# gnsscusdr/CU-SDR-Collection

Measured on AMD Instinct MI355X. Metric: IF Msamples/s through tracking correlators; x real-time @ 12-ch GPS L1 C/A, higher is better.
Workload: dtype f32 accumulate over int8 I/Q samples; f64/64-bit fixed-point code+carrier phase; 1 GPU; GPS L1 C/A, 12 channels/GPU, 1-ms E/P/L correlators, 60 s of int8 I/Q IF at 18 Msps (2.16 GB in HBM), batched replay of 719976 blocks per step; channels_per_gpu=12, epochs=59998

## Files before the change

cu-sdr-collection_amd/csrc/corr_common.h:

```cpp
#pragma once
#include <type_traits>

#include "gc_internal.h"


namespace gcorr {

constexpr int kWG = 256;
constexpr int kSPL = 8;

enum Mode { I8_IQ = 0, I8_QI, I16_IQ, I16_QI, I8_REAL, I16_REAL };

constexpr int kInlineBlocks = 16;
constexpr int kGuard = 16;

template <int ARMS>
struct ArmPitch {
  static constexpr int v = ARMS == 1 ? 1 : ARMS == 2 ? 2 : 4;
};
inline int gc_arm_pitch(int arms) { return arms <= 1 ? 1 : arms == 2 ? 2 : 4; }

constexpr int kLaneWaves = 16;

constexpr int kLaneReseedSteps = 128;

__host__ __device__ inline unsigned int gc_tie_window_units(double max_ramp, int lane_steps) {
  const int drift = lane_steps <= kLaneReseedSteps ? lane_steps : kLaneReseedSteps + lane_steps / kLaneReseedSteps + 1;
  return 2u + (unsigned int)drift + (unsigned int)(max_ramp * (16.0 * 2.220446049250313e-16 * 4294967296.0));
}

__host__ __device__ inline unsigned int gc_tie_window_units6(double max_ramp, int lane_steps, double m6) {
  const int drift = lane_steps <= kLaneReseedSteps ? lane_steps : kLaneReseedSteps + lane_steps / kLaneReseedSteps + 1;
  return (unsigned int)(m6 * (double)(4 + drift)) + 8u + (unsigned int)(max_ramp * (16.0 * 2.220446049250313e-16 * 4294967296.0));
}

struct TaggedSlot {
  double value;
  unsigned int tag;
  unsigned int zero;
};

struct InlineBlocks {
  gc_block b[kInlineBlocks];
};

struct DevLoopArgs;

struct KArgs {
  const uint8_t* if_base;
  const gc_block* blocks;
  const DevChannel* chans;
  double* out;
  double* partial;
  double fs;
  double inv_fs;
  int64_t nblocks;
  int splits;
  int xcd_swizzle;
  int red_off;
  int bpw;
  int stride;
  TaggedSlot* tagged;
  unsigned int notify_tag;
  int use_inline;
  const struct DevLoopArgs* devloop;
  int wide;
  long long total_wg;
  int share_el;
  int derived;
  int rho_off;
};

struct Fx {
  int k0;
  unsigned long long G;
};

__device__ __forceinline__ unsigned long long frac_to_u64(double g) {
  const double gh = g * 4294967296.0;
  const unsigned int hi = (unsigned int)gh;
  const double gl = (gh - (double)hi) * 4294967296.0;
  const unsigned int lo = (unsigned int)gl;
  return ((unsigned long long)hi << 32) | lo;
}

__device__ __forceinline__ Fx to_fx(double t) {
  const double kf = ceil(t);
  Fx r;
  r.k0 = (int)kf;
  r.G = frac_to_u64(kf - t);
  return r;
}

template <int MODE>
__device__ __forceinline__ void load_chunk(const uint8_t* __restrict__ base, long long q,
                                           float (&a)[kSPL], float (&b)[kSPL]) {
  if constexpr (MODE == I8_IQ || MODE == I8_QI) {
    const uint4 v = *reinterpret_cast<const uint4*>(base + 16 * q);
    const unsigned int w[4] = {v.x, v.y, v.z, v.w};
#pragma unroll
    for (int j = 0; j < kSPL; ++j) {
      const unsigned int word = w[j >> 1];
      const int sh = (j & 1) * 16;
      const float x0 = (float)(int)(signed char)(word >> sh);
      const float x1 = (float)(int)(signed char)(word >> (sh + 8));
      a[j] = (MODE == I8_IQ) ? x0 : x1;
      b[j] = (MODE == I8_IQ) ? x1 : x0;
    }
  } else if constexpr (MODE == I16_IQ || MODE == I16_QI) {
    const uint4 v0 = *reinterpret_cast<const uint4*>(base + 32 * q);
    const uint4 v1 = *reinterpret_cast<const uint4*>(base + 32 * q + 16);
    const unsigned int w[8] = {v0.x, v0.y, v0.z, v0.w, v1.x, v1.y, v1.z, v1.w};
#pragma unroll
    for (int j = 0; j < kSPL; ++j) {
      const float x0 = (float)(int)(short)(w[j] & 0xffffu);
      const float x1 = (float)(int)(short)(w[j] >> 16);
      a[j] = (MODE == I16_IQ) ? x0 : x1;
      b[j] = (MODE == I16_IQ) ? x1 : x0;
    }
  } else if constexpr (MODE == I8_REAL) {
    const uint2 v = *reinterpret_cast<const uint2*>(base + 8 * q);
    const unsigned int w[2] = {v.x, v.y};
#pragma unroll
    for (int j = 0; j < kSPL; ++j) {
      a[j] = (float)(int)(signed char)(w[j >> 2] >> ((j & 3) * 8));
      b[j] = 0.0f;
    }
  } else {
    const uint4 v = *reinterpret_cast<const uint4*>(base + 16 * q);
    const unsigned int w[4] = {v.x, v.y, v.z, v.w};
#pragma unroll
    for (int j = 0; j < kSPL; ++j) {
      a[j] = (float)(int)(short)((w[j >> 1] >> ((j & 1) * 16)) & 0xffffu);
      b[j] = 0.0f;
    }
  }
}

template <int MODE>
struct Fmt {
  static constexpr int bps = (MODE == I8_IQ || MODE == I8_QI || MODE == I16_REAL) ? 2 : (MODE == I8_REAL) ? 1 : 4;
  static constexpr bool swap = (MODE == I8_QI || MODE == I16_QI);
};

template <int MODE, int SPL>
__device__ __forceinline__ void load_words(const uint8_t* __restrict__ base, long long q,
                                           unsigned int (&w)[SPL * Fmt<MODE>::bps / 4]) {
  constexpr int NW = SPL * Fmt<MODE>::bps / 4;
  const uint8_t* p = base + (long long)(SPL * Fmt<MODE>::bps) * q;
  if constexpr (NW == 2) {
    const uint2 v = *reinterpret_cast<const uint2*>(p);
    w[0] = v.x; w[1] = v.y;
  } else {
#pragma unroll
    for (int k = 0; k < NW / 4; ++k) {
      const uint4 v = *reinterpret_cast<const uint4*>(p + 16 * k);
      w[4 * k] = v.x; w[4 * k + 1] = v.y; w[4 * k + 2] = v.z; w[4 * k + 3] = v.w;
    }
  }
}

template <int MODE, int SPL>
__device__ __forceinline__ void mask_words(unsigned int (&w)[SPL * Fmt<MODE>::bps / 4], int i0, int N) {
  constexpr int bits = 8 * Fmt<MODE>::bps;
  constexpr int per_word = 32 / bits;
#pragma unroll
  for (int j = 0; j < SPL; ++j) {
    const bool valid = (unsigned int)(i0 + j) < (unsigned int)N;
    const unsigned int m = (bits == 32) ? 0xffffffffu : (((1u << bits) - 1u) << ((j % per_word) * bits));
    if (!valid) w[j / per_word] &= ~m;
  }
}

#define GC_CVT_SDWA(sel)                                                                                  \
  {                                                                                                       \
    float r;                                                                                              \
    asm("v_cvt_f32_i32_sdwa %0, sext(%1) dst_sel:DWORD dst_unused:UNUSED_PAD src0_sel:" sel : "=v"(r) : "v"(word)); \
    return r;                                                                                             \
  }
template <int B>
__device__ __forceinline__ float cvt_byte(unsigned int word) {
  if constexpr (B == 0) GC_CVT_SDWA("BYTE_0")
  else if constexpr (B == 1) GC_CVT_SDWA("BYTE_1")
  else if constexpr (B == 2) GC_CVT_SDWA("BYTE_2")
  else GC_CVT_SDWA("BYTE_3")
}
template <int H>
__device__ __forceinline__ float cvt_half(unsigned int word) {
  if constexpr (H == 0) GC_CVT_SDWA("WORD_0")
  else GC_CVT_SDWA("WORD_1")
}

template <int MODE, int J, int NW>
__device__ __forceinline__ void sample_ab(const unsigned int (&w)[NW], float& a, float& b) {
  float x0, x1;
  if constexpr (MODE == I8_IQ || MODE == I8_QI) {
    x0 = cvt_byte<(J & 1) * 2>(w[J >> 1]);
    x1 = cvt_byte<(J & 1) * 2 + 1>(w[J >> 1]);
  } else if constexpr (MODE == I16_IQ || MODE == I16_QI) {
    x0 = cvt_half<0>(w[J]);
    x1 = cvt_half<1>(w[J]);
  } else if constexpr (MODE == I8_REAL) {
    x0 = cvt_byte<J & 3>(w[J >> 2]);
    x1 = 0.0f;
  } else {
    x0 = cvt_half<J & 1>(w[J >> 1]);
    x1 = 0.0f;
  }
  a = Fmt<MODE>::swap ? x1 : x0;
  b = Fmt<MODE>::swap ? x0 : x1;
}

template <int J, int SPL, typename F>
__device__ __forceinline__ void static_for(F&& f) {
  if constexpr (J < SPL) {
    f(std::integral_constant<int, J>{});
    static_for<J + 1, SPL>(f);
  }
}

__device__ __forceinline__ float wave_sum_lane63(float v) {
  auto dpp = [](float x, auto ctrl, auto row_mask) {
    return __int_as_float(__builtin_amdgcn_update_dpp(0, __float_as_int(x), decltype(ctrl)::value,
                                                      decltype(row_mask)::value, 0xf, true));
  };
  v += dpp(v, std::integral_constant<int, 0x111>{}, std::integral_constant<int, 0xf>{});
  v += dpp(v, std::integral_constant<int, 0x112>{}, std::integral_constant<int, 0xf>{});
  v += dpp(v, std::integral_constant<int, 0x114>{}, std::integral_constant<int, 0xf>{});
  v += dpp(v, std::integral_constant<int, 0x118>{}, std::integral_constant<int, 0xf>{});
  v += dpp(v, std::integral_constant<int, 0x142>{}, std::integral_constant<int, 0xa>{});
  v += dpp(v, std::integral_constant<int, 0x143>{}, std::integral_constant<int, 0xc>{});
  return v;
}

#ifndef GC_LANE_PN
#define GC_LANE_PN 1
#endif

__device__ __forceinline__ int wave_transpose_slot(int lane) {
  return ((lane >> 2) & 3) | ((lane & 3) << 2) | (lane & 16);
}
namespace wts {
template <int CTRL>
__device__ __forceinline__ float quad(float x) {
  return __int_as_float(__builtin_amdgcn_update_dpp(0, __float_as_int(x), CTRL, 0xf, 0xf, true));
}
__device__ __forceinline__ float pick(float x, float y, unsigned long long mask) {
  float r;
  asm("v_cndmask_b32_e64 %0, %1, %2, %3" : "=v"(r) : "v"(x), "v"(y), "s"(mask));
  return r;
}
template <int S>
__device__ __forceinline__ float row_pair(float x, float y) {
  float r;
  if constexpr (S == 4)
    asm("s_nop 1\n\tv_add_f32_dpp %0, %1, %1 row_shl:4 row_mask:0xf bank_mask:0x5\n\t"
        "v_add_f32_dpp %0, %2, %2 row_shr:4 row_mask:0xf bank_mask:0xa"
        : "=&v"(r) : "v"(x), "v"(y));
  else
    asm("s_nop 1\n\tv_add_f32_dpp %0, %1, %1 row_shl:8 row_mask:0xf bank_mask:0x3\n\t"
        "v_add_f32_dpp %0, %2, %2 row_shr:8 row_mask:0xf bank_mask:0xc"
        : "=&v"(r) : "v"(x), "v"(y));
  return r;
}
}

template <int K>
__device__ __forceinline__ float wave_transpose_sum(const float (&v)[K], int lane) {
  static_assert(K >= 1 && K <= 32, "one value per lane of half a wave at most");
  constexpr int N1 = (K + 1) / 2, N2 = (N1 + 1) / 2, N3 = (N2 + 1) / 2, N4 = (N3 + 1) / 2;
  constexpr unsigned long long kBit0 = 0xaaaaaaaaaaaaaaaaull, kBit1 = 0xccccccccccccccccull, kBit4 = 0xffff0000ffff0000ull;
  float a1[N1], a2[N2], a3[N3], a4[N4];
#pragma unroll
  for (int i = 0; i < N1; ++i) a1[i] = wts::row_pair<4>(v[2 * i], v[2 * i + 1 < K ? 2 * i + 1 : 2 * i]);
#pragma unroll
  for (int i = 0; i < N2; ++i) a2[i] = wts::row_pair<8>(a1[2 * i], a1[2 * i + 1 < N1 ? 2 * i + 1 : 2 * i]);
#pragma unroll
  for (int i = 0; i < N3; ++i) {
    if (2 * i + 1 < N2)
      a3[i] = wts::pick(a2[2 * i], a2[2 * i + 1], kBit0) + wts::quad<0xB1>(wts::pick(a2[2 * i + 1], a2[2 * i], kBit0));
    else
      a3[i] = a2[2 * i] + wts::quad<0xB1>(a2[2 * i]);
  }
#pragma unroll
  for (int i = 0; i < N4; ++i) {
    if (2 * i + 1 < N3)
      a4[i] = wts::pick(a3[2 * i], a3[2 * i + 1], kBit1) + wts::quad<0x4E>(wts::pick(a3[2 * i + 1], a3[2 * i], kBit1));
    else
      a4[i] = a3[2 * i] + wts::quad<0x4E>(a3[2 * i]);
  }
  float r;
  if constexpr (N4 == 2)
    r = wts::pick(a4[0], a4[1], kBit4) + __int_as_float(__builtin_amdgcn_ds_swizzle(__float_as_int(wts::pick(a4[1], a4[0], kBit4)), 0x401F));
  else
    r = a4[0] + __int_as_float(__builtin_amdgcn_ds_swizzle(__float_as_int(a4[0]), 0x401F));
  return r + __int_as_float(__builtin_amdgcn_ds_bpermute((lane ^ 32) << 2, __float_as_int(r)));
}

__device__ __forceinline__ float rl_f(float v, int lane) {
  return __int_as_float(__builtin_amdgcn_readlane(__float_as_int(v), lane));
}
__device__ __forceinline__ unsigned int rl_u(unsigned int v, int lane) {
  return (unsigned int)__builtin_amdgcn_readlane((int)v, lane);
}


constexpr size_t kInlineOffset = (sizeof(KArgs) + 7) / 8 * 8;

__device__ __forceinline__ gc_block load_block(const KArgs& p, long long lb) {
#if defined(__HIP_DEVICE_COMPILE__)
  if (p.use_inline) {
    typedef const __attribute__((address_space(4))) char* cptr4;
    typedef const __attribute__((address_space(4))) unsigned long long* qptr4;
    qptr4 src = (qptr4)((cptr4)__builtin_amdgcn_kernarg_segment_ptr() + kInlineOffset + lb * sizeof(gc_block));
    union {
      gc_block b;
      unsigned long long q[sizeof(gc_block) / 8];
    } u;
#pragma unroll
    for (int i = 0; i < (int)(sizeof(gc_block) / 8); ++i) u.q[i] = src[i];
    return u.b;
  }
#endif
  return p.blocks[lb];
}


}

int gc_launch_devloop_lane(gc_context* ctx, const gcorr::KArgs& a, const LaunchScope& s, unsigned int grid, bool share_el, int waves);
int gc_launch_correlator_lane(gc_context* ctx, const gcorr::KArgs& a, const gcorr::InlineBlocks& ib, const LaunchScope& s, const LaunchPlan& plan);
int gc_launch_correlator_multi(gc_context* ctx, const gcorr::KArgs& a, const LaunchScope& s, const LaunchPlan& plan);
int gc_launch_correlator_cboc(gc_context* ctx, const gcorr::KArgs& a, const LaunchScope& s, const LaunchPlan& plan);
int gc_launch_devloop(gc_context* ctx, const gcorr::KArgs& a, const LaunchScope& s, unsigned int grid, bool spl16, bool share_el);
int gc_launch_correlator_fast(gc_context* ctx, const gcorr::KArgs& a, const gcorr::InlineBlocks& ib, const LaunchScope& s, const LaunchPlan& plan);
```

cu-sdr-collection_amd/csrc/corr_fast.hip:

```cpp
#include <cstdlib>

#include "corr_common.h"
#include "devloop.h"

using namespace gcorr;

namespace {

constexpr float kTieTol = 4e-6f;
constexpr int kFW = 64;
#ifndef GC_SCHED_GROUP
#define GC_SCHED_GROUP 4
#endif
#ifndef GC_FAST_PARENT_SCHEDULE
#define GC_FAST_PARENT_SCHEDULE 0
#endif

template <int OFF_RE, int OFF_IM>
__device__ __forceinline__ void store_prefix(float tr, float ti, unsigned int lds_base) {
  asm volatile("s_mov_b32 m0, %2\n\ts_nop 0\n\tds_write_addtid_b32 %0 offset:%3\n\tds_write_addtid_b32 %1 offset:%4"
               :
               : "v"(tr), "v"(ti), "s"(lds_base), "n"(OFF_RE), "n"(OFF_IM)
               : "memory", "m0");
}

__device__ __forceinline__ double half_sum_f64(double v) {
  auto dpp64 = [](double x, auto ctrl, auto row_mask) {
    const unsigned long long b = (unsigned long long)__double_as_longlong(x);
    const unsigned int lo = (unsigned int)__builtin_amdgcn_update_dpp(0, (int)(unsigned int)b, decltype(ctrl)::value, decltype(row_mask)::value, 0xf, true);
    const unsigned int hi = (unsigned int)__builtin_amdgcn_update_dpp(0, (int)(unsigned int)(b >> 32), decltype(ctrl)::value, decltype(row_mask)::value, 0xf, true);
    return __longlong_as_double((long long)(((unsigned long long)hi << 32) | lo));
  };
  v += dpp64(v, std::integral_constant<int, 0x111>{}, std::integral_constant<int, 0xf>{});
  v += dpp64(v, std::integral_constant<int, 0x112>{}, std::integral_constant<int, 0xf>{});
  v += dpp64(v, std::integral_constant<int, 0x114>{}, std::integral_constant<int, 0xf>{});
  v += dpp64(v, std::integral_constant<int, 0x118>{}, std::integral_constant<int, 0xf>{});
  v += dpp64(v, std::integral_constant<int, 0x142>{}, std::integral_constant<int, 0xa>{});
  return v;
}
__device__ __forceinline__ double rl_f64(double x, int lane) {
  const unsigned long long b = (unsigned long long)__double_as_longlong(x);
  return __longlong_as_double((long long)(((unsigned long long)(unsigned int)__builtin_amdgcn_readlane((int)(b >> 32), lane) << 32) |
                                          (unsigned int)__builtin_amdgcn_readlane((int)(unsigned int)b, lane)));
}

template <int ARMS, int MODE, int SPL, bool CL, bool SHARE_EL, int WIDE, bool DEVLOOP = false>
__global__ __launch_bounds__(WIDE != 0 ? 256 : kFW) void corr_epl_fast_kernel(const KArgs p, const InlineBlocks ) {
  extern __shared__ __attribute__((aligned(16))) unsigned char smem[];
  constexpr int NW = SPL * Fmt<MODE>::bps / 4;
  constexpr bool kReal = (MODE == I8_REAL || MODE == I16_REAL);
  constexpr int kShift = (SPL == 16) ? 4 : 3;

  long long wg = blockIdx.x;
  if (p.xcd_swizzle && !DEVLOOP) {
    const long long per = (long long)gridDim.x >> 3;
    wg = (wg & 7) * per + (wg >> 3);
    if (wg >= p.total_wg) return;
  }
  const int lane = threadIdx.x & 63;
  const int wave = WIDE != 0 ? __builtin_amdgcn_readfirstlane((int)(threadIdx.x >> 6)) : 0;
  const bool wave_items = WIDE != 0 && p.bpw == 1;
  const long long item = wave_items ? wg * 4 + wave : wg;
  const long long wq = (DEVLOOP && p.xcd_swizzle) ? (item & 7) + 8 * ((item >> 3) / p.splits) : item / p.splits;
  const int split = (DEVLOOP && p.xcd_swizzle) ? (int)((item >> 3) % p.splits) : (int)(item - wq * p.splits);
  const long long grp = wq / p.stride;
  const int cslot = (int)(wq - grp * p.stride);

  constexpr bool TABF = (WIDE == 2);
  float2* tab2[ARMS];
  unsigned short* tab16[ARMS];
  float* tabf[ARMS];
  {
    const long long lb0 = min(grp * p.bpw * p.stride + cslot, (long long)p.nblocks - 1);
    const gc_block blk0 = DEVLOOP ? p.devloop->chan[lb0].blk : CL ? load_block(p, lb0) : p.blocks[lb0];
    const DevChannel* __restrict__ chn0 = p.chans + blk0.channel;
#pragma unroll
    for (int a = 0; a < ARMS; ++a) {
      const int aa = (a < chn0->arms) ? a : 0;
      tab2[a] = reinterpret_cast<float2*>(smem + 8 * (size_t)chn0->lds_off[aa]);
      tab16[a] = reinterpret_cast<unsigned short*>(smem + 2 * (size_t)chn0->lds_off[aa]);
      tabf[a] = reinterpret_cast<float*>(smem + 4 * (size_t)chn0->lds_off[aa]);
      if (a < chn0->arms) {
        const int off = blk0.table_offset[a];
        const int n = min(chn0->stage_len[a], chn0->nent[a] - off);
        if constexpr (TABF) {
          const float2* __restrict__ src = chn0->tab2[a] + off;
#pragma unroll 4
          for (int i = threadIdx.x; i < n + 3; i += 256) tabf[a][i] = src[i].x;
          if (threadIdx.x == 0) tabf[a][n + 3] = 0.0f;
        } else if constexpr (WIDE != 0) {
          const unsigned short* __restrict__ src = chn0->tab2b[a] + off;
#pragma unroll 4
          for (int i = threadIdx.x; i < n + 3; i += 256) tab16[a][i] = src[i];
        } else {
          const float2* __restrict__ src = chn0->tab2[a] + off;
#pragma unroll 4
          for (int i = lane; i < n + 3; i += kFW) tab2[a][i] = src[i];
        }
      }
    }
    __syncthreads();
  }
  auto table_entry = [&](int ar, int k) -> float2 {
    if constexpr (TABF) {
      return make_float2(tabf[ar][k + 1], tabf[ar][k + 2]);
    } else if constexpr (WIDE != 0) {
      const unsigned int e = tab16[ar][k + 1];
      float c, dc;
      asm("v_cvt_f32_i32_sdwa %0, sext(%1) dst_sel:DWORD dst_unused:UNUSED_PAD src0_sel:BYTE_0" : "=v"(c) : "v"(e));
      asm("v_cvt_f32_i32_sdwa %0, sext(%1) dst_sel:DWORD dst_unused:UNUSED_PAD src0_sel:BYTE_1" : "=v"(dc) : "v"(e));
      return make_float2(c, dc);
    } else {
      return tab2[ar][k + 1];
    }
  };
  float* pfx = reinterpret_cast<float*>(smem + p.red_off + (DEVLOOP ? 8 * 3 * 64 : 64)) + (WIDE != 0 ? wave * SPL * 2 * kFW : 0);
  unsigned int pfx_m0 = __builtin_amdgcn_readfirstlane((unsigned int)(size_t)pfx);
  if (wave_items && wq >= p.nblocks) return;

  [[maybe_unused]] DevLoopArgs dl_loc;
  if constexpr (DEVLOOP) dl_loc = *p.devloop;
  int nloop = p.bpw;
  gc_block dl_next;
  (void)dl_next;
  DevLoopChan dl_st;
  if constexpr (DEVLOOP) dl_st = p.devloop->chan[min(wq, (long long)p.nblocks - 1)];
  (void)dl_st;
  if constexpr (DEVLOOP) nloop = dl_st.epoch_budget;
  constexpr int kPfWords = SPL * Fmt<MODE>::bps / 4;
  [[maybe_unused]] unsigned int pf_w[kPfWords];
  [[maybe_unused]] long long pf_off = -1;
  constexpr bool kLoadAfterWait = !CL && !DEVLOOP && GC_FAST_PARENT_SCHEDULE == 0;
  for (int bi = (WIDE != 0 && !wave_items) ? wave : 0; bi < nloop; bi += (WIDE != 0 && !wave_items) ? 4 : 1) {
  const long long lb = DEVLOOP ? wq : (grp * p.bpw + bi) * p.stride + cslot;
  if (lb >= p.nblocks) break;
  gc_block blk;
  if constexpr (DEVLOOP) {
    if (dl_loc.host_loop) {
      const DevLoopArgs* dl = &dl_loc;
      const msg_t* dm = (split == 0 ? dl->host_desc : dl->desc_msg) + lb * kDescWords;
      msg_t m = {0u, 0u, 0u, 0u};
      unsigned int spins = 0;
      while (true) {
        if (lane < kDescWords) m = msg_load(dm + lane);
        const bool ok = lane >= kDescWords || m.z == (unsigned int)bi + 1u || m.z == 0xffffffffu;
        if (__all(ok)) break;
        if (++spins > (1u << 22)) break;
        __builtin_amdgcn_s_sleep(2);
      }
      if (spins > (1u << 22)) {
        if (lane == 0) dl->chan[lb].status = 3;
        if (split == 0 && lane < kDescWords) msg_store(dl->desc_msg + lb * kDescWords + lane, msg_t{3u, 0u, (unsigned int)bi + 1u, 0u});
        break;
      }
      if (split == 0 && lane < kDescWords) msg_store(dl->desc_msg + lb * kDescWords + lane, m);
      union {
        gc_block b;
        unsigned long long q[sizeof(gc_block) / 8];
      } u;
#pragma unroll
      for (int i = 0; i < (int)(sizeof(gc_block) / 8); ++i)
        u.q[i] = ((unsigned long long)(unsigned int)__builtin_amdgcn_readlane((int)m.y, i) << 32) | (unsigned int)__builtin_amdgcn_readlane((int)m.x, i);
      if (__builtin_amdgcn_readlane((int)m.x, kDescWords - 1) != 0) break;
      blk = u.b;
    } else if (bi > 0) {
      blk = dl_next;
    } else {
      if (dl_st.status != 0) break;
      blk = dl_st.blk;
    }
  } else {
    blk = CL ? load_block(p, lb) : p.blocks[lb];
  }
  unsigned long long dl_t0 = 0;
  if constexpr (DEVLOOP) dl_t0 = __builtin_amdgcn_s_memrealtime();
  const DevChannel* __restrict__ chn = p.chans + blk.channel;
  const int arms_here = chn->arms;

  const double R = chn->index_scale;
  const double M = chn->mult[0];
  const double rem = blk.rem_code_phase;
  const double step = blk.code_phase_step;
  const double d = blk.el_spacing;
  const int N = blk.blksize;
  const long long s0 = blk.first_sample;
  const double aE = (rem - d) * R;
  const double aL = (rem + d) * R;
  const double aP = rem * R;
  const double sp = step * R;
  const double tau = blk.carr_freq * p.inv_fs;
  const double spM = sp * M;
  double rspM = __builtin_amdgcn_rcp(spM);
  rspM = fma(rspM, fma(-spM, rspM, 1.0), rspM);
  rspM = fma(rspM, fma(-spM, rspM, 1.0), rspM);
  const float uk = (float)(rspM * 2.3283064365386963e-10);
  const bool tie_free = __builtin_amdgcn_readfirstlane((int)(blk.reserved & 1)) != 0;

  float myC, myS;
  unsigned int myJlo, myJhi;
  int myJint;
  {
    const int j = (lane < SPL) ? lane : SPL * kFW;
    const double x = (double)j * tau;
    sincospif(2.0f * (float)(x - floor(x)), &myS, &myC);
    const double y = (double)j * (sp * M);
    const double yi = floor(y);
    const unsigned long long jf = frac_to_u64(y - yi);
    myJint = (int)yi;
    myJlo = (unsigned int)jf;
    myJhi = (unsigned int)(jf >> 32);
  }
  float C[SPL], S[SPL];
#pragma unroll
  for (int j = 0; j < SPL; ++j) {
    C[j] = rl_f(myC, j);
    S[j] = rl_f(myS, j);
  }
  const float rotC = rl_f(myC, SPL), rotS = rl_f(myS, SPL);
  const unsigned long long Df = ((unsigned long long)rl_u(myJhi, SPL) << 32) | rl_u(myJlo, SPL);
  const int Di = __builtin_amdgcn_readlane(myJint, SPL);

  const long long q0 = s0 >> kShift;
  const long long q1 = (s0 + N - 1) >> kShift;
  const int nchunks = (int)(q1 - q0 + 1);
  const int cps = (nchunks + p.splits - 1) / p.splits;
  const int cbeg = split * cps;
  const int cend = min(nchunks, cbeg + cps);

  float accr[ARMS][3], acci[ARMS][3];
#pragma unroll
  for (int a = 0; a < ARMS; ++a)
#pragma unroll
    for (int x = 0; x < 3; ++x) accr[a][x] = acci[a][x] = 0.0f;

  const int iters = (cend - cbeg + kFW - 1) / kFW;
  const int c0 = cbeg + lane;
  float wc = 1.0f, ws = 0.0f;
  if (iters > 0) {
    constexpr int CB = SPL * Fmt<MODE>::bps;
    const int i00 = (int)((q0 + c0) * SPL - s0);
    constexpr bool SHARE = SHARE_EL;
    constexpr int NS = SHARE ? 2 : 3;
    Fx fx[NS];
    const double isp = __dmul_rn((double)i00, sp);
    fx[0] = to_fx(__dmul_rn(__dadd_rn(aE, isp), M));
    fx[1] = to_fx(__dmul_rn(__dadd_rn(aP, isp), M));
    if constexpr (!SHARE) fx[2] = to_fx(__dmul_rn(__dadd_rn(aL, isp), M));
    const uint8_t* __restrict__ base = p.if_base;

    const bool share_broken = SHARE_EL && __builtin_amdgcn_readfirstlane(2.0 * d * R * M == 1.0 ? 0 : 1) != 0;
    unsigned int glo[NS], ghi[NS];
    int kk[NS];
#pragma unroll
    for (int sx = 0; sx < NS; ++sx) {
      glo[sx] = (unsigned int)fx[sx].G;
      ghi[sx] = (unsigned int)(fx[sx].G >> 32);
      kk[sx] = fx[sx].k0;
    }
    const unsigned int Dlo = (unsigned int)Df, Dhi = (unsigned int)(Df >> 32);
    const uint8_t* __restrict__ bs = base + (long long)CB * (q0 + cbeg);
    const unsigned int voff = (unsigned int)lane * CB;
    const unsigned int voff_last = min(voff, (unsigned int)(cend - 1 - cbeg - (iters - 1) * kFW) * CB);

    auto load_k = [&](const int k, unsigned int (&w)[NW]) {
      const uint8_t* __restrict__ pk = bs + (size_t)k * (size_t)(kFW * CB);
      const unsigned int off = (k == iters - 1) ? voff_last : voff;
      load_words<MODE, SPL>(pk + off, 0, w);
    };

    auto process = [&](unsigned int (&w)[NW], const int k) {
      const bool last = (k == iters - 1);
      if ((k == 0) | last) {
        int kq = k;
        asm volatile("" : "+v"(kq));
        const int i0 = i00 + kq * (SPL * kFW);
        if (last && c0 + kq * kFW >= cend) {
#pragma unroll
          for (int q = 0; q < NW; ++q) w[q] = 0u;
#pragma unroll
          for (int sx = 0; sx < NS; ++sx) kk[sx] = 0;
        }
        if ((i0 < 0) | (i0 + SPL > N)) mask_words<MODE, SPL>(w, i0, N);
      }

      float gh[NS];
#pragma unroll
      for (int sx = 0; sx < NS; ++sx) asm("v_cvt_f32_u32_e32 %0, %1" : "=v"(gh[sx]) : "v"(ghi[sx]));
      bool exact = share_broken;
      if (!tie_free) {
        bool suspect = false;
#pragma unroll
        for (int sx = 0; sx < NS; ++sx) {
          const float u = gh[sx] * uk;
          suspect |= fabsf(u - rintf(u)) < kTieTol;
        }
        exact |= __any(suspect) != 0;
      }

      float Ur[ARMS][3], Ui[ARMS][3];
      if (exact) {
#pragma unroll
        for (int ar = 0; ar < ARMS; ++ar)
#pragma unroll
          for (int x = 0; x < 3; ++x) Ur[ar][x] = Ui[ar][x] = 0.0f;
        {
          int kq = k, Nq = N;
          asm volatile("" : "+v"(kq), "+v"(Nq));
          const int c = c0 + kq * kFW;
          const bool act = c < cend;
          const int i0 = i00 + kq * (SPL * kFW);
          const double bP = __dmul_rn(__dadd_rn(__dmul_rn((double)(Nq - 1), step), rem), R);
          const double bE = __dmul_rn(__dadd_rn(__dadd_rn(__dmul_rn((double)(Nq - 1), step), rem), -d), R);
          const double bL = __dmul_rn(__dadd_rn(__dadd_rn(__dmul_rn((double)(Nq - 1), step), rem), d), R);
          const uint8_t* sp8 = base + (long long)CB * (q0 + min(c, cend - 1));
          float cr = 1.0f, ci = 0.0f;
#pragma unroll 1
          for (int j = 0; j < SPL; ++j) {
            const int i = i0 + j;
            float x0, x1 = 0.0f;
            if constexpr (Fmt<MODE>::bps == 2 && !kReal) {
              x0 = (float)(signed char)sp8[2 * j];
              x1 = (float)(signed char)sp8[2 * j + 1];
            } else if constexpr (Fmt<MODE>::bps == 4) {
              x0 = (float)reinterpret_cast<const short*>(sp8)[2 * j];
              x1 = (float)reinterpret_cast<const short*>(sp8)[2 * j + 1];
            } else if constexpr (Fmt<MODE>::bps == 1) {
              x0 = (float)(signed char)sp8[j];
            } else {
              x0 = (float)reinterpret_cast<const short*>(sp8)[j];
            }
            float a = Fmt<MODE>::swap ? x1 : x0, b = Fmt<MODE>::swap ? x0 : x1;
            if ((unsigned int)i >= (unsigned int)Nq || !act) a = b = 0.0f;
            const float yr = a * cr + b * ci;
            const float yi = b * cr - a * ci;
            const float ncr = cr * C[1] - ci * S[1], nci = cr * S[1] + ci * C[1];
            cr = ncr;
            ci = nci;
#pragma unroll
            for (int x = 0; x < 3; ++x) {
              const double ax = (x == 0) ? aE : (x == 1) ? aP : aL;
              const double bx = (x == 0) ? bE : (x == 1) ? bP : bL;
              double t;
              if (2 * i < Nq - 1)
                t = __dadd_rn(ax, __dmul_rn((double)i, sp));
              else if (2 * i > Nq - 1)
                t = __dadd_rn(bx, -__dmul_rn((double)(Nq - 1 - i), sp));
              else
                t = __dadd_rn(ax, bx) / 2.0;
              int kx = (int)ceil(__dmul_rn(t, M));
              kx = max(-1, min(kx, 0x3fffffff));
#pragma unroll
              for (int ar = 0; ar < ARMS; ++ar) {
                const int kc = min(kx, chn->stage_len[(ar < arms_here) ? ar : 0] + 1);
                const float cf = table_entry(ar, kc).x;
                Ur[ar][x] = fmaf(cf, yr, Ur[ar][x]);
                Ui[ar][x] = fmaf(cf, yi, Ui[ar][x]);
              }
            }
          }
        }
      } else {
        float Tr = 0.f, Ti = 0.f;
        static_for<0, SPL>([&](auto jc) {
          constexpr int j = decltype(jc)::value;
          if constexpr (j % GC_SCHED_GROUP == 0 && j != 0) __builtin_amdgcn_sched_barrier(0);
          float a, b;
          sample_ab<MODE, j, NW>(w, a, b);
          if constexpr (kReal) {
            Tr = fmaf(a, C[j], Tr);
            Ti = fmaf(-a, S[j], Ti);
          } else {
            Tr = fmaf(a, C[j], fmaf(b, S[j], Tr));
            Ti = fmaf(b, C[j], fmaf(-a, S[j], Ti));
          }
          store_prefix<(2 * j) * kFW * 4, (2 * j + 1) * kFW * 4>(Tr, Ti, pfx_m0);
        });
        float Sr[NS], Si[NS], Pr[NS], Pi[NS];
#pragma unroll
        for (int sx = 0; sx < NS; ++sx) {
          const int m = min((int)(gh[sx] * uk), SPL - 1);
          Pr[sx] = pfx[(2 * m) * kFW + lane];
          Pi[sx] = pfx[(2 * m + 1) * kFW + lane];
          Sr[sx] = Tr - Pr[sx];
          Si[sx] = Ti - Pi[sx];
        }
#pragma unroll
        for (int x = 0; x < 3; ++x) {
#pragma unroll
          for (int ar = 0; ar < ARMS; ++ar) {
            const int sx = (SHARE && x == 2) ? 0 : x;
            const float2 cd = table_entry(ar, kk[sx] + ((SHARE && x == 2) ? 1 : 0));
            Ur[ar][x] = fmaf(cd.x, TABF ? Pr[sx] : Tr, cd.y * Sr[sx]);
            Ui[ar][x] = fmaf(cd.x, TABF ? Pi[sx] : Ti, cd.y * Si[sx]);
          }
        }
      }
#pragma unroll
      for (int ar = 0; ar < ARMS; ++ar)
#pragma unroll
        for (int x = 0; x < 3; ++x) {
          const float nr = fmaf(accr[ar][x], rotC, fmaf(-acci[ar][x], rotS, Ur[ar][x]));
          const float ni = fmaf(accr[ar][x], rotS, fmaf(acci[ar][x], rotC, Ui[ar][x]));
          accr[ar][x] = nr;
          acci[ar][x] = ni;
        }
#pragma unroll
      for (int sx = 0; sx < NS; ++sx)
        asm("v_sub_co_u32_e32 %0, vcc, %0, %3\n\tv_subb_co_u32_e32 %1, vcc, %1, %4, vcc\n\tv_addc_co_u32_e32 %2, vcc, %2, %5, vcc"
            : "+v"(glo[sx]), "+v"(ghi[sx]), "+v"(kk[sx])
            : "v"(Dlo), "v"(Dhi), "v"(Di)
            : "vcc");
    };

    unsigned int wa[NW], wb[NW];
    bool fetched = false;
    if constexpr (DEVLOOP) {
      const long long want = (long long)CB * (q0 + cbeg) + (long long)((0 == iters - 1) ? voff_last : voff);
      fetched = __all(pf_off == want) != 0;
      if (fetched) {
#pragma unroll
        for (int q = 0; q < NW; ++q) wa[q] = pf_w[q];
      }
      pf_off = -1;
    }
    if (!fetched) load_k(0, wa);
    auto arrived = [&](unsigned int (&w)[NW]) {
      if constexpr (kLoadAfterWait) {
#pragma unroll
        for (int q = 0; q < NW; ++q) asm volatile("" : "+v"(w[q]));
        asm volatile("" : : : "memory");
      }
    };
    for (int k = 0;; k += 2) {
      arrived(wa);
      if (k + 1 < iters) load_k(k + 1, wb);
      process(wa, k);
      if (k + 1 >= iters) break;
      arrived(wb);
      if (k + 2 < iters) load_k(k + 2, wa);
      process(wb, k + 1);
      if (k + 2 >= iters) break;
    }
    const double ph = blk.rem_carr_phase * 0.15915494309189535 + (double)(i00 + (iters - 1) * (SPL * kFW)) * tau;
    sincospif(2.0f * (float)(ph - floor(ph)), &ws, &wc);
  }

#ifndef GC_FAST_F64_TOTALS
#define GC_FAST_F64_TOTALS 0
#endif
  constexpr bool kF64Tot = CL || DEVLOOP || GC_FAST_F64_TOTALS != 0;
  double* o = (p.splits == 1) ? p.out + lb * GC_OUT_STRIDE : p.partial + (lb * p.splits + split) * GC_OUT_STRIDE;
  float tot[ARMS * 6];
  [[maybe_unused]] double totd[ARMS * 6];
#pragma unroll
  for (int ar = 0; ar < ARMS; ++ar)
#pragma unroll
    for (int x = 0; x < 3; ++x) {
      const float vr = wc * accr[ar][x] + ws * acci[ar][x], vi = wc * acci[ar][x] - ws * accr[ar][x];
      if constexpr (kF64Tot) {
        const double hr = half_sum_f64((double)vr), hi = half_sum_f64((double)vi);
        totd[ar * 6 + 2 * x] = rl_f64(hr, 31) + rl_f64(hr, 63);
        totd[ar * 6 + 2 * x + 1] = rl_f64(hi, 31) + rl_f64(hi, 63);
        tot[ar * 6 + 2 * x] = (float)totd[ar * 6 + 2 * x];
        tot[ar * 6 + 2 * x + 1] = (float)totd[ar * 6 + 2 * x + 1];
      } else {
        tot[ar * 6 + 2 * x] = wave_sum_lane63(vr);
        tot[ar * 6 + 2 * x + 1] = wave_sum_lane63(vi);
      }
    }
  if constexpr (DEVLOOP) {
#if defined(GC_DEVLOOP_ARGS_BY_POINTER) && GC_DEVLOOP_ARGS_BY_POINTER
    const DevLoopArgs* dl = p.devloop;
#else
    const DevLoopArgs* dl = &dl_loc;
#endif
    const unsigned int tag = (unsigned int)bi + 1u;
    msg_t* pm = dl->part_msg + ((lb * 2 + (bi & 1)) * dl->splits) * 2;
    if (lane == 63) {
      msg_store(pm + split * 2, msg_t{__float_as_uint(tot[0]), __float_as_uint(tot[1]), __float_as_uint(tot[2]), tag}, dl->reserved);
      msg_store(pm + split * 2 + 1, msg_t{__float_as_uint(tot[3]), __float_as_uint(tot[4]), __float_as_uint(tot[5]), tag}, dl->reserved);
    }
    const unsigned long long dl_t1 = __builtin_amdgcn_s_memrealtime();
    const DevLoopPre dl_pre = devloop_pre(dl, dl_st, blk, 1.0);
    const int mk = lane & 31, mh = lane >> 5;
    const bool mine = mk < dl->splits;
    msg_t m = {0u, 0u, 0u, 0u};
    unsigned int spins = 0;
    while (true) {
      if (mine) m = msg_load(pm + 2 * mk + mh, dl->reserved);
      const bool ok = !mine || m.w == tag;
      if (__all(ok)) break;
      if (++spins > (1u << 22)) break;
      __builtin_amdgcn_s_sleep(1);
    }
    if (spins > (1u << 22)) {
      if (lane == 0) dl->chan[lb].status = 3;
      break;
    }
    const unsigned long long dl_t2 = __builtin_amdgcn_s_memrealtime();
    if (!dl->host_loop && dl->prefetch) {
      constexpr int CBn = SPL * Fmt<MODE>::bps;
      const long long s0n = blk.first_sample + blk.blksize;
      const long long q0n = s0n >> kShift, q1n = (s0n + blk.blksize - 1) >> kShift;
      const int nchn = (int)(q1n - q0n + 1);
      const int cpsn = (nchn + p.splits - 1) / p.splits;
      const int cbegn = split * cpsn, cendn = min(nchn, cbegn + cpsn);
      const int itersn = (cendn - cbegn + kFW - 1) / kFW;
      if (itersn > 0 && (unsigned long long)(s0n + blk.blksize + 2 * SPL) <= dl->if_nsamples) {
        const unsigned int voffn = (unsigned int)lane * CBn;
        const unsigned int vlastn = min(voffn, (unsigned int)(cendn - 1 - cbegn - (itersn - 1) * kFW) * CBn);
        pf_off = (long long)CBn * (q0n + cbegn) + (long long)((0 == itersn - 1) ? vlastn : voffn);
        load_words<MODE, SPL>(p.if_base + pf_off, 0, pf_w);
      }
    }
    double part[3] = {mine ? (double)__uint_as_float(m.x) : 0.0, mine ? (double)__uint_as_float(m.y) : 0.0,
                      mine ? (double)__uint_as_float(m.z) : 0.0};
#pragma unroll
    for (int v = 0; v < 3; ++v) part[v] = half_sum_f64(part[v]);
    double sums[6];
#pragma unroll
    for (int v = 0; v < 6; ++v) sums[v] = rl_f64(part[v % 3], v < 3 ? 31 : 63);
    if (dl->host_loop) {
      if (split == 0) {
        TaggedSlot* ts = reinterpret_cast<TaggedSlot*>(dl->host_tagged) + lb * GC_OUT_STRIDE;
        double mine = 0.0;
#pragma unroll
        for (int v = 0; v < 6; ++v) mine = (lane == v) ? sums[v] : mine;
        if (lane < 6) {
          TaggedSlot rec;
          rec.value = mine;
          rec.tag = tag;
          rec.zero = 0u;
          *reinterpret_cast<uint4*>(ts + lane) = *reinterpret_cast<const uint4*>(&rec);
        }
        __threadfence_system();
      }
      continue;
    }
    dl_next = blk;
    double dl_rv[GC_TRK_NFIELDS];
    const bool cno_member = split == (p.splits > 1 ? 1 : 0);
    const int st = devloop_post<1>(dl, dl_st, dl_next, bi, sums, 1, 1.0, dl_pre, [&](int f, double v) { dl_rv[f] = v; }, cno_member,
                                   cno_member && lane == 0 ? (long long)lb : -1LL);
    {
      const bool spread = !dl->one_writer && p.splits >= GC_TRK_PILOT_I_E + 2;
      if (spread || split == 0) devloop_commit(dl, dl->chan + lb, dl_st, lb, bi, dl_rv, 1, lane, split, spread);
    }
    if (split == 0) {
      if (dl->timing == 1 && lane == 0) {
        const unsigned long long dl_t3 = __builtin_amdgcn_s_memrealtime();
        DevLoopChan* cc = dl->chan + lb;
        cc->pad[0] += (double)(dl_t1 - dl_t0);
        cc->pad[1] += (double)(dl_t2 - dl_t1);
        cc->pad[2] += (double)(dl_t3 - dl_t2);
      }
    }
    if (st != 0) break;
  } else if (CL) {
    TaggedSlot* ts = p.tagged + (lb * p.splits + split) * GC_OUT_STRIDE;
    double mine = 0.0;
#pragma unroll
    for (int v = 0; v < ARMS * 6; ++v) mine = (lane == v) ? totd[v] : mine;
    if (lane < ARMS * 6) {
      TaggedSlot rec;
      rec.value = (lane < arms_here * 6) ? mine : 0.0;
      rec.tag = p.notify_tag;
      rec.zero = 0u;
      *reinterpret_cast<uint4*>(ts + lane) = *reinterpret_cast<const uint4*>(&rec);
    }
  } else if (lane == 63) {
#pragma unroll
    for (int v = 0; v < ARMS * 6; ++v) o[v] = (v < arms_here * 6) ? (kF64Tot ? totd[v] : (double)tot[v]) : 0.0;
    for (int v = ARMS * 6; v < GC_OUT_STRIDE; ++v) o[v] = 0.0;
  }
  }

}
template <int ARMS, int MODE, int SPL>
void launch_variant(gc_context* ctx, const KArgs& a, const InlineBlocks& ib, dim3 grid, size_t smem) {
  const bool cl = a.tagged != nullptr;
  const bool share = (ARMS == 1) && a.share_el != 0;
  if (a.wide == 2) {
    if constexpr (ARMS == 1 && (MODE == I8_IQ || MODE == I8_QI)) {
      if (share) hipLaunchKernelGGL((corr_epl_fast_kernel<ARMS, MODE, SPL, false, true, 2>), grid, dim3(256), smem, ctx->stream, a, ib);
      else hipLaunchKernelGGL((corr_epl_fast_kernel<ARMS, MODE, SPL, false, false, 2>), grid, dim3(256), smem, ctx->stream, a, ib);
    }
    return;
  }
  if (a.wide) {
    if constexpr (ARMS <= 2 && (MODE == I8_IQ || MODE == I8_QI)) {
      if constexpr (SPL == 8) {
        if (cl) hipLaunchKernelGGL((corr_epl_fast_kernel<ARMS, MODE, SPL, true, false, 1>), grid, dim3(256), smem, ctx->stream, a, ib);
        else if (share) hipLaunchKernelGGL((corr_epl_fast_kernel<ARMS, MODE, SPL, false, ARMS == 1, 1>), grid, dim3(256), smem, ctx->stream, a, ib);
        else hipLaunchKernelGGL((corr_epl_fast_kernel<ARMS, MODE, SPL, false, false, 1>), grid, dim3(256), smem, ctx->stream, a, ib);
      } else {
        if (share) hipLaunchKernelGGL((corr_epl_fast_kernel<ARMS, MODE, SPL, false, ARMS == 1, 1>), grid, dim3(256), smem, ctx->stream, a, ib);
        else hipLaunchKernelGGL((corr_epl_fast_kernel<ARMS, MODE, SPL, false, false, 1>), grid, dim3(256), smem, ctx->stream, a, ib);
      }
    }
    return;
  }
  if constexpr (ARMS == 1) {
    if (cl && share) hipLaunchKernelGGL((corr_epl_fast_kernel<ARMS, MODE, SPL, true, true, 0>), grid, dim3(kFW), smem, ctx->stream, a, ib);
    else if (cl) hipLaunchKernelGGL((corr_epl_fast_kernel<ARMS, MODE, SPL, true, false, 0>), grid, dim3(kFW), smem, ctx->stream, a, ib);
    else if (share) hipLaunchKernelGGL((corr_epl_fast_kernel<ARMS, MODE, SPL, false, true, 0>), grid, dim3(kFW), smem, ctx->stream, a, ib);
    else hipLaunchKernelGGL((corr_epl_fast_kernel<ARMS, MODE, SPL, false, false, 0>), grid, dim3(kFW), smem, ctx->stream, a, ib);
  } else {
    (void)share;
    if (cl) hipLaunchKernelGGL((corr_epl_fast_kernel<ARMS, MODE, SPL, true, false, 0>), grid, dim3(kFW), smem, ctx->stream, a, ib);
    else hipLaunchKernelGGL((corr_epl_fast_kernel<ARMS, MODE, SPL, false, false, 0>), grid, dim3(kFW), smem, ctx->stream, a, ib);
  }
}

template <int ARMS, int SPL>
int launch_fast_mode(gc_context* ctx, const KArgs& a, const InlineBlocks& ib, dim3 grid, size_t smem) {
  int mode;
  if (ctx->if_dtype == GC_I8)
    mode = ctx->if_layout == GC_IQ ? I8_IQ : ctx->if_layout == GC_QI ? I8_QI : I8_REAL;
  else
    mode = ctx->if_layout == GC_IQ ? I16_IQ : ctx->if_layout == GC_QI ? I16_QI : I16_REAL;
  switch (mode) {
    case I8_IQ: launch_variant<ARMS, I8_IQ, SPL>(ctx, a, ib, grid, smem); break;
    case I8_QI: launch_variant<ARMS, I8_QI, SPL>(ctx, a, ib, grid, smem); break;
    case I16_IQ: launch_variant<ARMS, I16_IQ, 8>(ctx, a, ib, grid, smem); break;
    case I16_QI: launch_variant<ARMS, I16_QI, 8>(ctx, a, ib, grid, smem); break;
    case I8_REAL: launch_variant<ARMS, I8_REAL, 8>(ctx, a, ib, grid, smem); break;
    default: launch_variant<ARMS, I16_REAL, 8>(ctx, a, ib, grid, smem); break;
  }
  GC_HIP(hipGetLastError());
  return GC_OK;
}

template <int MODE, int SPL>
int launch_devloop_one(gc_context* ctx, KArgs& a, const InlineBlocks& ib, dim3 grid, size_t smem, bool share) {
  void* args[2] = {(void*)&a, (void*)&ib};
  const void* fn = share ? (const void*)corr_epl_fast_kernel<1, MODE, SPL, false, true, 0, true>
                         : (const void*)corr_epl_fast_kernel<1, MODE, SPL, false, false, 0, true>;
  GC_PERSIST(gc_launch_persistent(ctx, fn, grid, dim3(kFW), args, (unsigned int)smem));
  return GC_OK;
}

int launch_devloop_mode(gc_context* ctx, KArgs& a, const InlineBlocks& ib, dim3 grid, size_t smem, bool share, bool spl16) {
  const int lay = ctx->if_layout;
  if (ctx->if_dtype == GC_I8 && lay != GC_REAL) {
    if (spl16) return lay == GC_QI ? launch_devloop_one<I8_QI, 16>(ctx, a, ib, grid, smem, share) : launch_devloop_one<I8_IQ, 16>(ctx, a, ib, grid, smem, share);
    return lay == GC_QI ? launch_devloop_one<I8_QI, 8>(ctx, a, ib, grid, smem, share) : launch_devloop_one<I8_IQ, 8>(ctx, a, ib, grid, smem, share);
  }
  if (ctx->if_dtype == GC_I8) return launch_devloop_one<I8_REAL, 8>(ctx, a, ib, grid, smem, share);
  if (lay == GC_REAL) return launch_devloop_one<I16_REAL, 8>(ctx, a, ib, grid, smem, share);
  return lay == GC_QI ? launch_devloop_one<I16_QI, 8>(ctx, a, ib, grid, smem, share) : launch_devloop_one<I16_IQ, 8>(ctx, a, ib, grid, smem, share);
}

}

int gc_launch_devloop(gc_context* ctx, const KArgs& a_in, const LaunchScope& s, unsigned int grid, bool spl16, bool share_el) {
  KArgs a = a_in;
  InlineBlocks ib;
  std::memset(&ib, 0, sizeof ib);
  a.red_off = 8 * s.lds_bytes;
  const size_t smem = (size_t)a.red_off + 8 * 3 * 64 + (size_t)16 * kFW * sizeof(float2);
  return launch_devloop_mode(ctx, a, ib, dim3(grid), smem, share_el, spl16 && ctx->if_dtype == GC_I8 && ctx->if_layout != GC_REAL);
}

int gc_launch_correlator_fast(gc_context* ctx, const KArgs& a_in, const InlineBlocks& ib, const LaunchScope& s, const LaunchPlan& plan) {
  KArgs a = a_in;
  a.red_off = (a.wide == 2 ? 4 : a.wide ? 2 : 8) * s.lds_bytes;
  const unsigned int grid = plan.grid;
  const int max_arms = s.max_arms;
  const bool wide = plan.chunk == 16;
  size_t smem = (size_t)a.red_off + 64 + (size_t)(a.wide ? 4 : 1) * (wide ? 16 : 8) * kFW * sizeof(float2);
  if (const char* e = GC_TUNE_ENV("GC_FAST_EXTRA_LDS")) smem += (size_t)std::atoi(e);
  if (wide) {
    switch (max_arms) {
      case 1: return launch_fast_mode<1, 16>(ctx, a, ib, dim3(grid), smem);
      case 2: return launch_fast_mode<2, 16>(ctx, a, ib, dim3(grid), smem);
      default: return launch_fast_mode<3, 16>(ctx, a, ib, dim3(grid), smem);
    }
  }
  switch (max_arms) {
    case 1: return launch_fast_mode<1, 8>(ctx, a, ib, dim3(grid), smem);
    case 2: return launch_fast_mode<2, 8>(ctx, a, ib, dim3(grid), smem);
    default: return launch_fast_mode<3, 8>(ctx, a, ib, dim3(grid), smem);
  }
}
```

Baseline: 323,700 IF Msamples/s (all channels active, all GPUs).

## Hoist per-channel params to workgroup, branch-free edge masking, fewer DPP and FMA ops

Adds a default-on edge path for the non-CL, non-devloop fast kernel. Channel parameters (index scale, multiplier, arm count, stage lengths) are loaded once per workgroup instead of per block. Edge masking is applied only on the first and last lane of a chunk, and the mask itself is built from a bitmap without branches. It also fuses the wave-reduction DPP broadcasts into inline asm and rewrites the accumulator rotation FMAs with SGPR operands. The risk is correctness: this assumes every block in a workgroup shares one channel and that only the chunk ends ever need masking.

New measurement: 332,300 IF Msamples/s (all channels active, all GPUs) (median of 6 runs). +2.7%, better.

```diff
diff --git a/cu-sdr-collection_amd/csrc/corr_common.h b/cu-sdr-collection_amd/csrc/corr_common.h
--- a/cu-sdr-collection_amd/csrc/corr_common.h
+++ b/cu-sdr-collection_amd/csrc/corr_common.h
@@ -160,16 +160,39 @@
   }
 }
 
+#ifndef GC_FAST_PARENT_EDGES
+#define GC_FAST_PARENT_EDGES 0
+#endif
+
 template <int MODE, int SPL>
-__device__ __forceinline__ void mask_words(unsigned int (&w)[SPL * Fmt<MODE>::bps / 4], int i0, int N) {
+__host__ __device__ __forceinline__ void mask_words(unsigned int (&w)[SPL * Fmt<MODE>::bps / 4], int i0, int N) {
   constexpr int bits = 8 * Fmt<MODE>::bps;
   constexpr int per_word = 32 / bits;
+#if GC_FAST_PARENT_EDGES
 #pragma unroll
   for (int j = 0; j < SPL; ++j) {
     const bool valid = (unsigned int)(i0 + j) < (unsigned int)N;
     const unsigned int m = (bits == 32) ? 0xffffffffu : (((1u << bits) - 1u) << ((j % per_word) * bits));
     if (!valid) w[j / per_word] &= ~m;
   }
+#else
+  static_assert(SPL <= 16 && SPL % per_word == 0, "the bitmap of a chunk's samples is built with 32-bit shifts");
+  const int lo = i0 >= 0 ? 0 : (i0 <= -SPL ? SPL : -i0);
+  const unsigned int left = (unsigned int)N - (unsigned int)i0;
+  const int hi_raw = i0 >= N ? 0 : (left >= (unsigned int)SPL ? SPL : (int)left);
+  const int hi = hi_raw > lo ? hi_raw : lo;
+  const unsigned int valid = (1u << hi) - (1u << lo);
+#pragma unroll
+  for (int q = 0; q < SPL / per_word; ++q) {
+    unsigned int m = 0u;
+#pragma unroll
+    for (int s = 0; s < per_word; ++s) {
+      const unsigned int field = (bits == 32) ? 0xffffffffu : (((1u << bits) - 1u) << (s * bits));
+      m |= (0u - ((valid >> (q * per_word + s)) & 1u)) & field;
+    }
+    w[q] &= m;
+  }
+#endif
 }
 
 #define GC_CVT_SDWA(sel)                                                                                  \
@@ -228,8 +251,14 @@
   v += dpp(v, std::integral_constant<int, 0x112>{}, std::integral_constant<int, 0xf>{});
   v += dpp(v, std::integral_constant<int, 0x114>{}, std::integral_constant<int, 0xf>{});
   v += dpp(v, std::integral_constant<int, 0x118>{}, std::integral_constant<int, 0xf>{});
+#if GC_FAST_PARENT_EDGES
   v += dpp(v, std::integral_constant<int, 0x142>{}, std::integral_constant<int, 0xa>{});
   v += dpp(v, std::integral_constant<int, 0x143>{}, std::integral_constant<int, 0xc>{});
+#else
+  asm("s_nop 1\n\tv_add_f32_dpp %0, %0, %0 row_bcast:15 row_mask:0xa bank_mask:0xf\n\t"
+      "s_nop 1\n\tv_add_f32_dpp %0, %0, %0 row_bcast:31 row_mask:0xc bank_mask:0xf"
+      : "+v"(v));
+#endif
   return v;
 }
 
diff --git a/cu-sdr-collection_amd/csrc/corr_fast.hip b/cu-sdr-collection_amd/csrc/corr_fast.hip
--- a/cu-sdr-collection_amd/csrc/corr_fast.hip
+++ b/cu-sdr-collection_amd/csrc/corr_fast.hip
@@ -50,6 +50,7 @@
   constexpr int NW = SPL * Fmt<MODE>::bps / 4;
   constexpr bool kReal = (MODE == I8_REAL || MODE == I16_REAL);
   constexpr int kShift = (SPL == 16) ? 4 : 3;
+  constexpr bool kEdges = !CL && !DEVLOOP && GC_FAST_PARENT_EDGES == 0;
 
   long long wg = blockIdx.x;
   if (p.xcd_swizzle && !DEVLOOP) {
@@ -70,13 +71,21 @@
   float2* tab2[ARMS];
   unsigned short* tab16[ARMS];
   float* tabf[ARMS];
+  [[maybe_unused]] double wg_R = 0.0, wg_M = 0.0;
+  [[maybe_unused]] int wg_arms = 0, wg_stage[ARMS];
   {
     const long long lb0 = min(grp * p.bpw * p.stride + cslot, (long long)p.nblocks - 1);
     const gc_block blk0 = DEVLOOP ? p.devloop->chan[lb0].blk : CL ? load_block(p, lb0) : p.blocks[lb0];
     const DevChannel* __restrict__ chn0 = p.chans + blk0.channel;
+    if constexpr (kEdges) {
+      wg_R = chn0->index_scale;
+      wg_M = chn0->mult[0];
+      wg_arms = chn0->arms;
+    }
 #pragma unroll
     for (int a = 0; a < ARMS; ++a) {
       const int aa = (a < chn0->arms) ? a : 0;
+      if constexpr (kEdges) wg_stage[a] = chn0->stage_len[aa];
       tab2[a] = reinterpret_cast<float2*>(smem + 8 * (size_t)chn0->lds_off[aa]);
       tab16[a] = reinterpret_cast<unsigned short*>(smem + 2 * (size_t)chn0->lds_off[aa]);
       tabf[a] = reinterpret_cast<float*>(smem + 4 * (size_t)chn0->lds_off[aa]);
@@ -174,11 +183,19 @@
   }
   unsigned long long dl_t0 = 0;
   if constexpr (DEVLOOP) dl_t0 = __builtin_amdgcn_s_memrealtime();
-  const DevChannel* __restrict__ chn = p.chans + blk.channel;
-  const int arms_here = chn->arms;
-
-  const double R = chn->index_scale;
-  const double M = chn->mult[0];
+  [[maybe_unused]] const DevChannel* __restrict__ chn = p.chans + blk.channel;
+  int arms_here;
+  if constexpr (kEdges) arms_here = wg_arms;
+  else arms_here = chn->arms;
+
+  double R, M;
+  if constexpr (kEdges) {
+    R = wg_R;
+    M = wg_M;
+  } else {
+    R = chn->index_scale;
+    M = chn->mult[0];
+  }
   const double rem = blk.rem_code_phase;
   const double step = blk.code_phase_step;
   const double d = blk.el_spacing;
@@ -257,7 +274,10 @@
       ghi[sx] = (unsigned int)(fx[sx].G >> 32);
       kk[sx] = fx[sx].k0;
     }
-    const unsigned int Dlo = (unsigned int)Df, Dhi = (unsigned int)(Df >> 32);
+    const unsigned int Dlo = (unsigned int)Df;
+    unsigned int Dhi = (unsigned int)(Df >> 32);
+    int Di_v = Di;
+    if constexpr (kEdges) asm("" : "+v"(Dhi), "+v"(Di_v));
     const uint8_t* __restrict__ bs = base + (long long)CB * (q0 + cbeg);
     const unsigned int voff = (unsigned int)lane * CB;
     const unsigned int voff_last = min(voff, (unsigned int)(cend - 1 - cbeg - (iters - 1) * kFW) * CB);
@@ -280,7 +300,21 @@
 #pragma unroll
           for (int sx = 0; sx < NS; ++sx) kk[sx] = 0;
         }
-        if ((i0 < 0) | (i0 + SPL > N)) mask_words<MODE, SPL>(w, i0, N);
+        if constexpr (kEdges) {
+          if (k == 0) {
+            const int ih = __builtin_amdgcn_readlane(i0, 0);
+            if (ih < 0 && lane == 0) mask_words<MODE, SPL>(w, ih, N);
+          }
+          if (last) {
+            int ce = cend;
+            asm volatile("" : "+s"(ce));
+            const int tl = (ce - 1 - cbeg) & (kFW - 1);
+            const int it = __builtin_amdgcn_readlane(i0, tl);
+            if (it + SPL > N && lane == tl) mask_words<MODE, SPL>(w, it, N);
+          }
+        } else {
+          if ((i0 < 0) | (i0 + SPL > N)) mask_words<MODE, SPL>(w, i0, N);
+        }
       }
 
       float gh[NS];
@@ -351,7 +385,10 @@
               kx = max(-1, min(kx, 0x3fffffff));
 #pragma unroll
               for (int ar = 0; ar < ARMS; ++ar) {
-                const int kc = min(kx, chn->stage_len[(ar < arms_here) ? ar : 0] + 1);
+                int slen;
+                if constexpr (kEdges) slen = wg_stage[ar];
+                else slen = chn->stage_len[(ar < arms_here) ? ar : 0];
+                const int kc = min(kx, slen + 1);
                 const float cf = table_entry(ar, kc).x;
                 Ur[ar][x] = fmaf(cf, yr, Ur[ar][x]);
                 Ui[ar][x] = fmaf(cf, yi, Ui[ar][x]);
@@ -399,16 +436,23 @@
       for (int ar = 0; ar < ARMS; ++ar)
 #pragma unroll
         for (int x = 0; x < 3; ++x) {
-          const float nr = fmaf(accr[ar][x], rotC, fmaf(-acci[ar][x], rotS, Ur[ar][x]));
-          const float ni = fmaf(accr[ar][x], rotS, fmaf(acci[ar][x], rotC, Ui[ar][x]));
-          accr[ar][x] = nr;
-          acci[ar][x] = ni;
+          if constexpr (kEdges) {
+            const float tr = fmaf(-acci[ar][x], rotS, Ur[ar][x]);
+            asm("v_fma_f32 %0, %0, %1, %2" : "+v"(acci[ar][x]) : "s"(rotC), "v"(Ui[ar][x]));
+            acci[ar][x] = fmaf(accr[ar][x], rotS, acci[ar][x]);
+            asm("v_fma_f32 %0, %0, %1, %2" : "+v"(accr[ar][x]) : "s"(rotC), "v"(tr));
+          } else {
+            const float nr = fmaf(accr[ar][x], rotC, fmaf(-acci[ar][x], rotS, Ur[ar][x]));
+            const float ni = fmaf(accr[ar][x], rotS, fmaf(acci[ar][x], rotC, Ui[ar][x]));
+            accr[ar][x] = nr;
+            acci[ar][x] = ni;
+          }
         }
 #pragma unroll
       for (int sx = 0; sx < NS; ++sx)
         asm("v_sub_co_u32_e32 %0, vcc, %0, %3\n\tv_subb_co_u32_e32 %1, vcc, %1, %4, vcc\n\tv_addc_co_u32_e32 %2, vcc, %2, %5, vcc"
             : "+v"(glo[sx]), "+v"(ghi[sx]), "+v"(kk[sx])
-            : "v"(Dlo), "v"(Dhi), "v"(Di)
+            : "v"(Dlo), "v"(Dhi), "v"(Di_v)
             : "vcc");
     };
 
```
